# KangWelly/Assignment-for-AAE6102_GNSS-SDR

Measured on AMD Instinct MI355X. Metric: correlator Msamples/s (acq+track), whole job, higher is better.
Workload: dtype int8 in; acquisition: f64 correlation + f64 fine search; tracking: f64

## Files before the change

assignment-for-aae6102_gnss-sdr_amd/abi.py:

```python
from __future__ import annotations

import ctypes as C
import os
import sys

MAX_SV = 64
MAX_TAPS = 32

OK, ENODATA, EIO, EARG, EDEVICE, EINDEX = 0, 1, 2, 3, 4, 5

FIELDS = ["P_i", "P_q", "E_i", "E_q", "L_i", "L_q", "PLLdiscri", "DLLdiscri", "codedelay",
          "remChip", "codeFreq", "carrierFreq", "remPhase", "remSample", "numSample",
          "delayValue", "absoluteSample", "codedelay2"]
NFIELDS = len(FIELDS)
OUT_DEVICE = 1
FIELDS_POS = ["P_i", "P_q", "E_i", "E_q", "L_i", "L_q", "carrError", "codeError", "codedelay",
              "remChip", "codeFreq", "carrFreq", "remCarrPhase", "absoluteSampleCodedelay",
              "numSample", "delayValue", "absoluteSample", "codedelay2"]

MC_TAPS = 25
MC_TAP_NAMES = ([f"E_{{}}{s}" for s in ["_060", "_055", "", "_045", "_040", "_035", "_030", "_025",
                                         "_020", "_015", "_010", "_005"]] + ["P_{}"] +
                [f"L_{{}}{s}" for s in ["005", "010", "015", "020", "025", "030", "035", "040", "045",
                                         "", "055", "060"]])
# ... 319 lines not shown
                                    C.POINTER(GnssAcfOut)]),
    "gnss_acf_fit": (C.c_int, [C.c_void_p, C.POINTER(GnssAcfFitCfg), C.POINTER(GnssTrackOut), C.c_int32,
                               C.POINTER(GnssAcfFitOut)]),
    "gnss_acf_fit_window": (C.c_int, [C.POINTER(GnssAcfFitCfg), C.POINTER(C.c_double), C.POINTER(C.c_double),
                                      C.POINTER(GnssAcfFitOut)]),
    "gnss_lane_boundaries": (C.c_int, [C.POINTER(C.c_double), C.POINTER(C.c_double), C.c_int, C.c_int, C.c_double]),
    "gnss_ctx_lane_path": (C.c_int, [C.c_void_p]),
}

LIB_PATH = os.path.join(os.path.dirname(os.path.abspath(__file__)), "lib", "libgnss_mi355x.so")
_lib = None
_torch_first = False
LOADED_PATH = None

(OPT_FORCE_SUB, OPT_NO_PERSIST, OPT_FORCE_VPB, OPT_ACQ_ROCFFT, OPT_FINE_ROCFFT, OPT_ACQ_BATCH, OPT_ACQ_FUSED,
 OPT_ACQ_RING, OPT_ACQ_PIPE, OPT_VT_BLOCKS, OPT_FORCE_PEER, OPT_VT_SPAN, OPT_SLOT_PATH) = range(13)
MAX_DEVICES = 16


def require_torch():
    import torch
    if _lib is not None and not _torch_first:
        raise RuntimeError("import torch before the first gnss Context / abi.load() "
                           "(PyTorch-ROCm must bring up its HIP runtime first)")
    return torch


class GnssError(RuntimeError):
    def __init__(self, status, msg=""):
        self.status = status
        super().__init__(f"gnss status {status}: {msg}")
# ... 31 lines not shown
```

assignment-for-aae6102_gnss-sdr_amd/csrc/acq_fft.hip:

```cpp
#include "gnss_internal.h"

#pragma clang fp contract(fast)

namespace gnss {

namespace {

constexpr int kRow = 2000;
constexpr int kRowPad = 2100;
constexpr int kRowThreads = 256;
constexpr int kColThreads = 256;

template <int P> struct PrimeTab;
template <> struct PrimeTab<13> {
    static constexpr double c[13] = {1.0, 0.8854560256532099, 0.5680647467311559, 0.120536680255323, -0.35460488704253545, -0.7485107481711012, -0.970941817426052, -0.9709418174260521, -0.7485107481711013, -0.3546048870425359, 0.1205366802553232, 0.5680647467311548, 0.88545602565321};
    static constexpr double s[13] = {0.0, 0.4647231720437685, 0.8229838658936564, 0.992708874098054, 0.9350162426854148, 0.6631226582407952, 0.23931566428755768, -0.23931566428755743, -0.663122658240795, -0.9350162426854147, -0.992708874098054, -0.822983865893657, -0.4647231720437684};
};
template <> struct PrimeTab<29> {
    static constexpr double c[29] = {1.0, 0.9766205557100867, 0.907575419670957, 0.7960930657056438, 0.6473862847818277, 0.46840844069979015, 0.26752833852922075, 0.05413890858541761, -0.16178199655276473, -0.37013815533991423, -0.5611870653623823, -0.7259954919231306, -0.8568571761675893, -0.9476531711828025, -0.9941379571543596, -0.9941379571543597, -0.9476531711828025, -0.8568571761675892, -0.7259954919231311, -0.5611870653623825, -0.37013815533991445, -0.16178199655276476, 0.0541389085854167, 0.2675283385292201, 0.4684084406997903, 0.6473862847818279, 0.796093065705644, 0.9075754196709569, 0.9766205557100867};
    static constexpr double s[29] = {0.0, 0.21497044021102407, 0.4198891015602646, 0.6051742151937652, 0.7621620551276365, 0.8835120444460229, 0.963549992519223, 0.9985334138511238, 0.9868265225415261, 0.9289767198167915, 0.8276889981568906, 0.6876994588534235, 0.5155538571770216, 0.3193015301359798, 0.10811901842394192, -0.10811901842394124, -0.31930153013597995, -0.5155538571770218, -0.6876994588534231, -0.8276889981568905, -0.9289767198167914, -0.9868265225415261, -0.9985334138511239, -0.9635499925192231, -0.8835120444460228, -0.7621620551276362, -0.6051742151937649, -0.41988910156026493, -0.21497044021102438};
};

template <class V> struct RealOf;
template <> struct RealOf<float2> { using T = float; };
// ... 905 lines not shown
    t[e] = tw_row[t2 ? 10 * i * k : i * k];
}

__device__ __forceinline__ int64_t fine_code_of(int64_t n, double invFs, double invFc, double codelength)
{
    const double cvi = floor((invFs * (double)(n + 1)) / invFc);
    return (int64_t)fmod(cvi, codelength);
}

#ifndef GNSS_FINE_PREP
#define GNSS_FINE_PREP 1
#endif
#ifndef GNSS_FINE_TWIK
#define GNSS_FINE_TWIK 1
#endif
template <class Src> struct SrcElem;
template <> struct SrcElem<SrcIQ8> {
    using T = char2;
    static constexpr int kTM = 32;
    __device__ static T get(const SrcIQ8& s, int64_t n) { return reinterpret_cast<const char2*>(s.p)[n]; }
    static SrcIQ8 wrap(const T* p) { return SrcIQ8{reinterpret_cast<const int8_t*>(p)}; }
};
template <> struct SrcElem<SrcC64> {
    using T = double2;
    static constexpr int kTM = 8;
    __device__ static T get(const SrcC64& s, int64_t n) { return s.p[n]; }
    static SrcC64 wrap(const T* p) { return SrcC64{p}; }
};
template <int P, class Src>
__global__ __launch_bounds__(kRowThreads) void fine_prep_kernel(
    const Src src, const int32_t* __restrict__ cd, int64_t S, double invFs, double invFc, double codelength,
    const float* __restrict__ ca0, typename SrcElem<Src>::T* __restrict__ xt0, float* __restrict__ ct0)
{
    using T = typename SrcElem<Src>::T;
    constexpr int PT = P * kFineT, TM = SrcElem<Src>::kTM;
    constexpr int64_t M = (int64_t)PT * kRow;
    __shared__ T s_x[TM * PT];
    __shared__ float s_c[TM * PT];
    const float* ca = ca0 + (int64_t)blockIdx.y * 1023;
    const int m0 = blockIdx.x * TM, tid = threadIdx.x;
    const int tm = kRow - m0 < TM ? kRow - m0 : TM;
    const int64_t base = S - cd[blockIdx.y] - 1, n0 = (int64_t)PT * m0;
    for (int e = tid; e < tm * PT; e += kRowThreads) {
        s_x[e] = SrcElem<Src>::get(src, base + n0 + e);
        s_c[e] = ca[fine_code_of(n0 + e, invFs, invFc, codelength)];
    }
    __syncthreads();
    T* xt = xt0 + (int64_t)blockIdx.y * M;
    float* ct = ct0 + (int64_t)blockIdx.y * M;
    for (int e = tid; e < tm * PT; e += kRowThreads) {
        const int rho = e / tm, c = e - rho * tm;
        xt[(int64_t)rho * kRow + m0 + c] = s_x[c * PT + rho];
        ct[(int64_t)rho * kRow + m0 + c] = s_c[c * PT + rho];
    }
}

template <int P, class Src>
__global__ __launch_bounds__(kRowThreads) void fine_rows_kernel(
    const Src src, const float* __restrict__ ct, const int32_t* __restrict__ cd, int64_t S,
    const float* __restrict__ ca0, double invFs, double invFc, double codelength, int D, int64_t N,
    const double2* __restrict__ tw_row, const double2* __restrict__ twik, const double2* __restrict__ tabA,
    const double2* __restrict__ tabB, double2* __restrict__ E0)
{
    constexpr int T = kFineT;
    const int64_t base = S - cd[blockIdx.z] - 1;
    const float* ca = ca0 + (int64_t)blockIdx.z * 1023;
    double2* E = E0 + (int64_t)blockIdx.z * N;
    __shared__ double2 s_a[kRowPad];
    const int rho = blockIdx.x, r = blockIdx.y, tid = threadIdx.x;
    const int m2 = rho / P, n2 = rho - m2 * P;
    auto sample = [&](int m1) { return (int64_t)P * T * m1 + (int64_t)P * m2 + n2; };
    auto code_of = [&](int64_t n) { return fine_code_of(n, invFs, invFc, codelength); };
    if constexpr (GNSS_FINE_PREP) {
        constexpr int NIT = (kRow + kRowThreads - 1) / kRowThreads;
        const int64_t row0 = ((int64_t)blockIdx.z * P * T + rho) * kRow;
        double2 raw[NIT], ta[NIT];
        float cv[NIT];
#pragma unroll
        for (int q = 0; q < NIT; q++) {
            const int m10 = tid + q * kRowThreads, m1 = m10 < kRow ? m10 : kRow - 1;
            cv[q] = ct[row0 + m1];
// ... 49 lines not shown
        fft2000_r20first_put<-1>(s_a, tw_row, tid, put);
}

struct FineBest {
    double m;
    int64_t i;
};

__device__ __forceinline__ void best_merge(double& m, int64_t& i, double m2, int64_t i2)
{
    if (m2 > m || (m2 == m && i2 < i)) { m = m2; i = i2; }
}

template <int P>
__global__ __launch_bounds__(kColThreads) void fine_cols_kernel(
    const double2* __restrict__ E0, int D, int64_t N, int shifted, const double2* __restrict__ tabK,
    const double2* __restrict__ tabS, FineBest* __restrict__ part0)
{
    constexpr int T = kFineT, JC = kFineJC;
    const double2* E = E0 + (int64_t)blockIdx.z * N;
    FineBest* part = part0 + (int64_t)blockIdx.z * gridDim.x * gridDim.y;
    static_assert(P * T * JC * sizeof(double2) + (kColThreads / 64) * sizeof(double) * 2 <= 80 * 1024,
                  "fine_cols LDS tile: two blocks per CU of gfx950's 160 KiB");
    __shared__ double2 s_e[P * T * JC];
    __shared__ FineBest s_b[kColThreads / 64];
    const int r = blockIdx.y, j10 = blockIdx.x * JC, tid = threadIdx.x;
    auto at = [&](int e) {
        const int jj = e % JC, nm = e / JC;
        return E + ((int64_t)r * P * T + nm) * kRow + j10 + jj;
    };
    if constexpr (GNSS_STAGED_LOADS) {
        constexpr int NE = P * T * JC, NIT = (NE + kColThreads - 1) / kColThreads;
        double2 st[NIT];
#pragma unroll
// ... 40 lines not shown
    }
#pragma unroll
    for (int o = 32; o > 0; o >>= 1) {
        const double m2 = __shfl_xor(bm, o, 64);
        const int64_t i2 = __shfl_xor(bi, o, 64);
        best_merge(bm, bi, m2, i2);
    }
    if ((tid & 63) == 0) s_b[tid >> 6] = FineBest{bm, bi};
    __syncthreads();
    if (tid == 0) {
        for (int w = 1; w < kColThreads / 64; w++) best_merge(bm, bi, s_b[w].m, s_b[w].i);
        part[(int64_t)r * gridDim.x + blockIdx.x] = FineBest{bm, bi};
    }
}

__global__ void fine_best_final_kernel(const FineBest* __restrict__ part0, int nblk,
                                       int64_t* __restrict__ kbest0)
{
    const FineBest* part = part0 + (int64_t)blockIdx.x * nblk;
    int64_t* kbest = kbest0 + blockIdx.x;
    double bm = -1.0;
    int64_t bi = INT64_MAX;
    for (int k = threadIdx.x; k < nblk; k += blockDim.x) best_merge(bm, bi, part[k].m, part[k].i);
#pragma unroll
    for (int o = 32; o > 0; o >>= 1) {
        const double m2 = __shfl_xor(bm, o, 64);
        const int64_t i2 = __shfl_xor(bi, o, 64);
        best_merge(bm, bi, m2, i2);
    }
    __shared__ FineBest s_b[4];
    if ((threadIdx.x & 63) == 0) s_b[threadIdx.x >> 6] = FineBest{bm, bi};
    __syncthreads();
    if (threadIdx.x == 0) {
        for (int w = 1; w < (int)(blockDim.x >> 6); w++) best_merge(bm, bi, s_b[w].m, s_b[w].i);
        *kbest = bi + 1;
    }
}

}

bool acq_fft_supported(int64_t S) { return S == 13 * kRow || S == 29 * kRow; }

template <class V>
hipError_t launch_acq_fft_forward(const int8_t* iq, const double2* xs, int64_t S, int datalen, int nbins,
                                  double IF, double freqMin, double freqStep, double Fs, const float* ca,
                                  int nprn, double codeFreqBasis, const V* tw_row,
                                  const V* tw_col, V* B, V* X, hipStream_t s, int bin0, int nbc, bool codes)
{
    const int nsig = datalen * nbins;
    if (nbc < 0) nbc = nbins - bin0;
    if (bin0 < 0 || nbc < 0 || bin0 + nbc > nbins) return hipErrorInvalidValue;
// ... 136 lines not shown
};
FineLayout fine_layout(int64_t S, int L, int datalen)
{
    FineLayout f;
    f.M = (int64_t)L * S;
    f.N = f.M * datalen;
    f.tabs = kRow + (int64_t)kRow * datalen + (int64_t)kFineT * kRow + S + f.M / kRow + kTwIK;
    f.slab = f.N;
    f.part = (int64_t)datalen * (kRow / kFineJC);
    return f;
}
}

static size_t fine_prep_offset(const FineLayout& f, int nsv)
{
    const size_t b = sizeof(double2) * (size_t)(f.tabs + (int64_t)nsv * f.slab) + sizeof(FineBest) * (size_t)(nsv * f.part);
    return (b + 255) & ~(size_t)255;
}
size_t fine_fft_scratch_bytes(int64_t S, int L, int datalen, int nsv)
{
    const FineLayout f = fine_layout(S, L, datalen);
    if (!GNSS_FINE_PREP) return fine_prep_offset(f, nsv);
    return fine_prep_offset(f, nsv) + (size_t)nsv * f.M * (sizeof(double2) + sizeof(float));
}

hipError_t launch_fine_fft_tables(int64_t S, int L, int datalen, void* scratch, hipStream_t s)
{
    const int64_t M = (int64_t)L * S;
    double2* tw_row = static_cast<double2*>(scratch);
    double2* tabA = tw_row + kRow;
    double2* tabB = tabA + (int64_t)kRow * datalen;
    double2* tabK = tabB + (int64_t)kFineT * kRow;
    double2* tabS = tabK + S;
    const int64_t lens[5] = {kRow, (int64_t)kRow * datalen, (int64_t)kFineT * kRow, S, M / kRow};
    const int64_t divs[5] = {kRow, (int64_t)kRow * datalen, (int64_t)kFineT * kRow, M, M / kRow};
    const int64_t rows[5] = {0, kRow, kRow, kRow, 0};
    double2* tabs[5] = {tw_row, tabA, tabB, tabK, tabS};
    for (int t = 0; t < 5; t++)
        hipLaunchKernelGGL(fine_twiddle_kernel, dim3((unsigned)((lens[t] + 255) / 256)), dim3(256), 0,
                           s, tabs[t], lens[t], divs[t], rows[t]);
    hipLaunchKernelGGL(fine_twik_kernel, dim3((kTwIK + 255) / 256), dim3(256), 0, s, tw_row, tabS + M / kRow);
    return hipGetLastError();
}

hipError_t launch_fine_fft_argmax(const int8_t* iq, const double2* xs, int64_t S, int L, int datalen,
                                  const int32_t* cd, int nsv, const float* ca, double Fs, double codeFreqBasis,
                                  double codelength, int shifted, void* scratch, int64_t* kbest, hipStream_t s)
{
    if (nsv < 1 || nsv > 65535) return hipErrorInvalidValue;
    const FineLayout f = fine_layout(S, L, datalen);
    const int64_t N = f.N;
    double2* tw_row = static_cast<double2*>(scratch);
    double2* tabA = tw_row + kRow;
    double2* tabB = tabA + (int64_t)kRow * datalen;
    double2* tabK = tabB + (int64_t)kFineT * kRow;
    double2* tabS = tabK + S;
    double2* E = tw_row + f.tabs;
    FineBest* part = reinterpret_cast<FineBest*>(E + (int64_t)nsv * f.slab);
    char* prep = static_cast<char*>(scratch) + fine_prep_offset(f, nsv);
    float* ct = reinterpret_cast<float*>(prep + (size_t)nsv * f.M * sizeof(double2));
    const int nblk = kRow / kFineJC;
    auto rows = [&](auto src, auto* xt, auto kern, auto prep_kern, int tm) {
        using SrcT = decltype(src);
        if (GNSS_FINE_PREP) {
            hipLaunchKernelGGL(prep_kern, dim3((kRow + tm - 1) / tm, nsv), dim3(kRowThreads), 0, s, src, cd, S, 1 / Fs,
                               1 / codeFreqBasis, codelength, ca, xt, ct);
            src = SrcElem<SrcT>::wrap(xt);
        }
        hipLaunchKernelGGL(kern, dim3((unsigned)(f.M / kRow), datalen, nsv), dim3(kRowThreads), 0, s, src, ct, cd, S,
                           ca, 1 / Fs, 1 / codeFreqBasis, codelength, datalen, N, tw_row, tabS + f.M / kRow, tabA,
                           tabB, E);
    };
#define GNSS_FINE(P_)                                                                           \
    if (S == (int64_t)P_ * kRow) {                                                              \
        if (xs)                                                                                 \
            rows(SrcC64{xs}, reinterpret_cast<double2*>(prep), fine_rows_kernel<P_, SrcC64>,    \
                 fine_prep_kernel<P_, SrcC64>, SrcElem<SrcC64>::kTM);                           \
        else                                                                                    \
            rows(SrcIQ8{iq}, reinterpret_cast<char2*>(prep), fine_rows_kernel<P_, SrcIQ8>,      \
                 fine_prep_kernel<P_, SrcIQ8>, SrcElem<SrcIQ8>::kTM);                           \
        hipLaunchKernelGGL(fine_cols_kernel<P_>, dim3(nblk, datalen, nsv), dim3(kColThreads), 0, s, E, \
                           datalen, N, shifted, tabK, tabS, part);                                    \
        hipLaunchKernelGGL(fine_best_final_kernel, dim3(nsv), dim3(256), 0, s, part, nblk * datalen, \
                           kbest);                                                              \
        return hipGetLastError();                                                               \
    }
    GNSS_FINE(13) GNSS_FINE(29)
#undef GNSS_FINE
    return hipErrorInvalidValue;
}

}
```

assignment-for-aae6102_gnss-sdr_amd/csrc/api_acq.cpp:

```cpp
#include <cmath>
#include <cstring>
#include <vector>

#include "host.h"

using namespace gnss;
using namespace gnss::host;

namespace {
constexpr int kAcqPipeDefault = 2;
#ifndef GNSS_ACQ_FWD_SPLIT
#define GNSS_ACQ_FWD_SPLIT 1
#endif
constexpr bool kAcqFwdSplit = GNSS_ACQ_FWD_SPLIT;
constexpr int kAcqPairFront = 60;
constexpr int kFineBatch = 16;

template <class V> struct CplxReal;
template <> struct CplxReal<float2> { using T = float; };
template <> struct CplxReal<double2> { using T = double; };

template <class V>
int acq_search(gnss_ctx* ctx, const int8_t* blk, const double2* xa, int64_t S, int dl, int nb, int np,
               const gnss_signal* sg, const gnss_acq* acq, const float* ca, typename CplxReal<V>::T* corr,
// ... 145 lines not shown
    for (int p0 = 0; p0 < np; p0 += chunk) {
        const int pc = std::min(chunk, np - p0);
        if ((st = get_plan(ctx, S, (size_t)pc * nsig, dbl, 1, &pl))) return st;
    }
    HIP_TRY(hipEventRecord(e_all.a, ctx->stream));
    HIP_TRY(launch_acq_wipe(blk, xa, S, dl, nb, sg->IF, acq->freqMin, acq->freqStep, sg->Fs, sig.as<V>(), ctx->stream));
    if ((st = run_fft(ctx, sig.p, S, nsig, dbl, 0))) return st;
    HIP_TRY(launch_acq_code(ca, nullptr, np, S, sg->codeFreqBasis, sg->Fs, code.as<V>(), ctx->stream));
    if ((st = run_fft(ctx, code.p, S, np, dbl, 0))) return st;
    for (int p0 = 0; p0 < np; p0 += chunk) {
        const int pc = std::min(chunk, np - p0);
        HIP_TRY(launch_acq_mul(code.as<V>() + (size_t)p0 * S, sig.as<V>(), pc, nsig, S, y.as<V>(), ctx->stream));
        if ((st = run_fft(ctx, y.p, S, (size_t)pc * nsig, dbl, 1))) return st;
        HIP_TRY(launch_acq_power(y.as<V>(), pc, nb, dl, S, 0, corr + (size_t)p0 * nb * S, ctx->stream));
    }
    return GNSS_OK;
}
}

static int group_acquisition(gnss_ctx* g, const gnss_file* file, const gnss_signal* sg, const gnss_acq* acq,
                             gnss_acquired* out, gnss_acq_diag* diag)
{
    if (!file || !sg || !acq || !out) return GNSS_EARG;
    memset(out, 0, sizeof(*out));
    if (diag) memset(diag, 0, sizeof(*diag));
    g->timing = gnss_timing{};
    std::vector<int32_t> prns;
    if (acq->n_prn > 0 && acq->prn_list) prns.assign(acq->prn_list, acq->prn_list + acq->n_prn);
    else for (int i = 1; i <= 32; i++) prns.push_back(i);
    if (prns.size() > GNSS_MAX_SV) return fail(g, GNSS_EARG, "too many PRNs");
// ... 84 lines not shown
                                     xs_sums.as<unsigned long long>() + 2, ctx->stream));
        HIP_TRY(hipEventRecord(e_conv.b, ctx->stream));
    }
    const double2* xa = iq8 ? nullptr : xs_acq.as<double2>();
    const double2* xf = iq8 ? nullptr : xs_fine.as<double2>();

    std::vector<float> cah((size_t)np * 1023);
    for (int i = 0; i < np; i++) generate_ca(prns[i], &cah[(size_t)i * 1023]);
    DevBuf ca, corr, peaks, scratch;
    HIP_TRY(ca.alloc(ctx, "acq.ca", cah.size() * sizeof(float)));
    HIP_TRY(hipMemcpyAsync(ca.p, cah.data(), cah.size() * sizeof(float), hipMemcpyHostToDevice, ctx->stream));
    const int dbl = ctx->acq_fp64 ? 1 : 0;
    HIP_TRY(corr.alloc(ctx, "acq.corr", (dbl ? sizeof(double) : sizeof(float)) * (size_t)np * nb * S));
    HIP_TRY(peaks.alloc(ctx, "acq.peaks", sizeof(AcqPeak) * (size_t)np));
    HIP_TRY(scratch.alloc(ctx, "acq.scratch", acq_scratch_bytes(np, np)));
    Events e_all, e_corr;
    int perm = 0;
    DevBuf fsync;
    if (dbl)
        st = acq_search<double2>(ctx, blk, xa, S, dl, nb, np, sg, acq, ca.as<float>(), corr.as<double>(), e_all,
                                 &perm, fsync);
    else
        st = acq_search<float2>(ctx, blk, xa, S, dl, nb, np, sg, acq, ca.as<float>(), corr.as<float>(), e_all,
                                &perm, fsync);
    if (st) return st;
    const int cshift = (int)std::ceil(sg->Fs / sg->codeFreqBasis);
    if (dbl)
        HIP_TRY(launch_acq_peak(corr.as<double>(), np, nb, S, cshift, perm, peaks.as<AcqPeak>(), scratch.p,
                                ctx->stream));
    else
        HIP_TRY(launch_acq_peak(corr.as<float>(), np, nb, S, cshift, perm, peaks.as<AcqPeak>(), scratch.p,
                                ctx->stream));
    HIP_TRY(hipEventRecord(e_corr.b, ctx->stream));
    std::vector<AcqPeak> ph((size_t)np);
    HIP_TRY(hipMemcpyAsync(ph.data(), peaks.p, sizeof(AcqPeak) * (size_t)np, hipMemcpyDeviceToHost, ctx->stream));
    unsigned fused_err = 0;
    if (fsync.p)
        HIP_TRY(hipMemcpyAsync(&fused_err, static_cast<char*>(fsync.p) + acq_fused_err_offset(), sizeof(unsigned),
                               hipMemcpyDeviceToHost, ctx->stream));
    HIP_TRY(hipStreamSynchronize(ctx->stream));
    if (fused_err)
        return fail(ctx, GNSS_EDEVICE, "fused correlator: a pipeline wait timed out (grid not resident)");
    ctx->timing.acq_hypothesis_samples = (int64_t)np * nb * dl * S;

    std::vector<int> acq_idx;
    for (int i = 0; i < np; i++) {
        if (diag) {
            int k = diag->n++;
            diag->prn[k] = prns[i];
            diag->SNR[k] = ph[i].snr;
            diag->fbin[k] = ph[i].fbin + 1;
            diag->codePhase[k] = ph[i].cp + 1;
            diag->peak[k] = ph[i].peak;
            diag->peak2[k] = ph[i].peak2;
        }
        if (ph[i].snr >= 12) {
            int k = out->n++;
            out->sv[k] = prns[i];
            out->SNR[k] = ph[i].snr;
            out->Doppler[k] = acq->freqMin + acq->freqStep * (double)ph[i].fbin;
            out->codedelay[k] = ph[i].cp;
            acq_idx.push_back(i);
        }
    }
    if (out->n == 0) {
        HIP_TRY(hipEventRecord(e_all.b, ctx->stream));
        HIP_TRY(hipEventSynchronize(e_all.b));
        ctx->timing.acq_ms = e_all.ms();
        ctx->timing.acq_corr_ms = ctx->timing.acq_ms;
        return fail(ctx, GNSS_ENODATA, "No satellites acquired");
    }

    if (flen < off + S * bps * (L + 1)) return fail(ctx, GNSS_EIO, "IF record too short for fine search");
    const int fshift = dtyp == 2 ? 1 : 2;
    const int na = out->n;
    const int64_t N = (int64_t)L * S * dl;
    if (N % 2) return fail(ctx, GNSS_EINDEX, "odd fftlength: MATLAB indexes past the end (:116)");
    std::vector<float> caf((size_t)na * 1023);
    std::vector<int32_t> cdh((size_t)na);
    for (int k = 0; k < na; k++) {
        generate_ca(out->sv[k], &caf[(size_t)k * 1023]);
        cdh[k] = out->codedelay[k];
    }
    DevBuf fca, fcd, fx, kb;
    HIP_TRY(fca.alloc(ctx, "acq.fca", caf.size() * sizeof(float)));
    HIP_TRY(fcd.alloc(ctx, "acq.fcd", cdh.size() * sizeof(int32_t)));
    HIP_TRY(kb.alloc(ctx, "acq.kb", sizeof(int64_t) * (size_t)na));
    HIP_TRY(hipMemcpyAsync(fca.p, caf.data(), caf.size() * sizeof(float), hipMemcpyHostToDevice, ctx->stream));
    HIP_TRY(hipMemcpyAsync(fcd.p, cdh.data(), cdh.size() * sizeof(int32_t), hipMemcpyHostToDevice, ctx->stream));
    const bool own_fine = fine_fft_supported(S, L) && !ctx->opt[GNSS_OPT_FINE_ROCFFT];
    Events e_fine;
    if (own_fine) {
        const int fb = std::min(na, kFineBatch);
        HIP_TRY(fx.alloc(ctx, "acq.fx", fine_fft_scratch_bytes(S, L, dl, fb)));
        HIP_TRY(hipEventRecord(e_fine.a, ctx->stream));
        HIP_TRY(launch_fine_fft_tables(S, L, dl, fx.p, ctx->stream));
        for (int k0 = 0; k0 < na; k0 += fb) {
            const int nk = std::min(fb, na - k0);
            HIP_TRY(launch_fine_fft_argmax(blk, xf, S, L, dl, fcd.as<int32_t>() + k0, nk,
                                           fca.as<float>() + (size_t)k0 * 1023, sg->Fs, sg->codeFreqBasis,
                                           sg->codelength, fshift, fx.p, kb.as<int64_t>() + k0, ctx->stream));
        }
    } else {
        HIP_TRY(fx.alloc(ctx, "acq.fx", sizeof(double2) * (size_t)na * N));
        rocfft_plan pl;
        if ((st = get_plan(ctx, N, na, 1, 0, &pl))) return st;
        HIP_TRY(hipEventRecord(e_fine.a, ctx->stream));
        HIP_TRY(launch_fine_build(blk, xf, S, L, fcd.as<int32_t>(), fca.as<float>(), na, sg->Fs, sg->codeFreqBasis,
                                  sg->codelength, N, fx.as<double2>(), ctx->stream));
        if ((st = run_fft(ctx, fx.p, N, na, 1, 0))) return st;
        DevBuf fscr;
        HIP_TRY(fscr.alloc(ctx, "acq.fscr", acq_scratch_bytes(1, na)));
        HIP_TRY(launch_fine_argmax(fx.as<double2>(), na, N, fshift, fscr.p, kb.as<int64_t>(), ctx->stream));
    }
    HIP_TRY(hipEventRecord(e_fine.b, ctx->stream));
    HIP_TRY(hipEventRecord(e_all.b, ctx->stream));
    std::vector<int64_t> kh((size_t)na);
    HIP_TRY(hipMemcpyAsync(kh.data(), kb.p, sizeof(int64_t) * (size_t)na, hipMemcpyDeviceToHost, ctx->stream));
    HIP_TRY(hipStreamSynchronize(ctx->stream));
    for (int k = 0; k < na; k++) {
        const double K = (double)kh[k];
        out->fineFreq[k] = (file->dataType == 2) ? (-K * (sg->Fs / (double)N) + sg->Fs / 2) : (K * (sg->Fs / (double)N));
    }
    {
        float f = 0;
        (void)hipEventElapsedTime(&f, e_all.a, e_corr.b);
        ctx->timing.acq_corr_ms = f;
    }
    ctx->timing.acq_fine_ms = e_fine.ms();
    ctx->timing.acq_ms = e_all.ms() + (iq8 ? 0.0 : e_conv.ms());
    return GNSS_OK;
}

}
// ... 1 lines not shown
```

assignment-for-aae6102_gnss-sdr_amd/csrc/gnss_internal.h:

```cpp
#pragma once

#include <hip/hip_runtime.h>
#include <stdint.h>

#include "../../include/gnss_mi355x.h"

#define GNSS_HD __host__ __device__ __forceinline__

namespace gnss {

struct Colon {
    double a, d, c;
    int64_t n;
};

GNSS_HD Colon colon_make(double a, double d, double b)
{
    Colon r{a, d, b, -1};
    if (!(a - a == 0) || !(d - d == 0) || !(b - b == 0)) return r;
    if (d == 0 || (a < b && d < 0) || (b < a && d > 0)) return r;
    double tol = 2.0 * 2.220446049250313e-16 * fmax(fabs(a), fabs(b));
    double sig = d > 0 ? 1.0 : -1.0;
    double n;
    if (a == floor(a) && d == 1) {
// ... 400 lines not shown
hipError_t launch_acq_fft_correlate(const double2* C, const double2* X, int64_t S, int datalen,
                                    int nbins, int nprn, int first_pair, int npair,
                                    const double2* tw_row, const double2* tw_col, double2* A,
                                    double* corr, hipStream_t s, int parts = kAcqCols | kAcqRows);
hipError_t launch_acq_fft_pair(const double2* C, const double2* X, int64_t S, int datalen, int nbins, int nprn,
                               int cols_first, int cols_n, double2* Acols, int rows_first, int rows_n,
                               const double2* Arows, const double2* tw_row, const double2* tw_col, double* corr,
                               int front, hipStream_t s);
size_t acq_fused_sync_bytes();
size_t acq_fused_err_offset();
size_t acq_fused_ring_bytes(int64_t S);
hipError_t launch_acq_fft_correlate_fused(const double2* C, const double2* X, int64_t S, int datalen, int nbins,
                                          int nprn, int nslot, const double2* tw_row, const double2* tw_col,
                                          double2* ring, void* sync, double* corr, hipStream_t s);
bool fine_fft_supported(int64_t S, int L);
size_t fine_fft_scratch_bytes(int64_t S, int L, int datalen, int nsv);
hipError_t launch_fine_fft_tables(int64_t S, int L, int datalen, void* scratch, hipStream_t s);
hipError_t launch_fine_fft_argmax(const int8_t* iq, const double2* xs, int64_t S, int L, int datalen,
                                  const int32_t* cd, int nsv, const float* ca, double Fs, double codeFreqBasis,
                                  double codelength, int shifted, void* scratch, int64_t* kbest, hipStream_t s);
hipError_t launch_fine_build(const int8_t* iq, const double2* xs, int64_t S, int L, const int32_t* codedelay,
                             const float* ca, int nsv, double Fs, double codeFreqBasis,
                             double codelength, int64_t N, double2* out, hipStream_t s);
hipError_t launch_fine_argmax(const double2* F, int nsv, int64_t N, int shifted, void* scratch,
                              int64_t* kbest, hipStream_t s);

size_t acq_scratch_bytes(int nprn, int nsv);

hipError_t launch_stage_cpx(const int8_t* src, int prec, int type, int64_t nsamp, double2* out,
                            unsigned long long* sums, hipStream_t s);
hipError_t launch_real8_to_iq8(const int8_t* src, int64_t n, int8_t* dst, hipStream_t s);
size_t prefix16_scratch_bytes(int64_t ngroups);
hipError_t launch_prefix16(const short* src, int64_t ngroups, long long* pref_i, long long* pref_q,
                           void* scratch, size_t scratch_bytes, hipStream_t s);

// ... 265 lines not shown
```

assignment-for-aae6102_gnss-sdr_amd/csrc/host.h:

```cpp
#pragma once

#include <hip/hip_runtime.h>
#include <rocfft/rocfft.h>

#include <algorithm>
#include <cstdint>
#include <cstdlib>
#include <map>
#include <string>
#include <thread>
#include <tuple>
#include <utility>
#include <vector>

#include "gnss_internal.h"
#include "group.h"

struct gnss_ctx {
    int device = 0;
    hipStream_t stream = nullptr;
    hipStream_t stream2 = nullptr;
    hipEvent_t ev_cols[2] = {}, ev_rows[2] = {};
    std::string err;
    gnss_timing timing{};
    int profiling = 0;
    std::map<std::tuple<size_t, size_t, int, int>, rocfft_plan> plans;
    void* fft_work = nullptr;
    size_t fft_work_size = 0;
    std::map<std::string, std::pair<void*, size_t>> pool;
    std::map<std::string, std::pair<void*, size_t>> pinned;
    int64_t acq_tw_S = 0;
    int acq_tw_dbl = -1;
    int acq_fp64 = 1;
    uint64_t window = 0;
    int64_t opt[GNSS_OPT_COUNT] = {};
    int lane_path = 0;
    std::vector<gnss_ctx*> members;
    bool member = false;
    int fail_chan = -1;
    gnss::group::ResidentCache<void*> resident;
};

namespace gnss {
namespace host {

inline const char* probe_env(const char* name)
{
// ... 136 lines not shown
```

include/gnss_mi355x.h:

```cpp
#ifndef GNSS_MI355X_H
#define GNSS_MI355X_H

#include <stdint.h>
#include <stddef.h>

#ifdef __cplusplus
extern "C" {
#endif

#define GNSS_ABI_VERSION 13

#define GNSS_OK         0
#define GNSS_ENODATA    1
#define GNSS_EIO        2
#define GNSS_EARG       3
#define GNSS_EDEVICE    4
#define GNSS_EINDEX     5

#define GNSS_MAX_SV     64
#define GNSS_MAX_TAPS   32


typedef struct gnss_file {
    const char   *path;
// ... 119 lines not shown
int  gnss_ctx_set_acq_precision(gnss_ctx *ctx, int fp64);
int  gnss_ctx_set_window(gnss_ctx *ctx, uint64_t bytes);
#define GNSS_OPT_FORCE_SUB    0
#define GNSS_OPT_NO_PERSIST   1
#define GNSS_OPT_FORCE_VPB    2
#define GNSS_OPT_ACQ_ROCFFT   3
#define GNSS_OPT_FINE_ROCFFT  4
#define GNSS_OPT_ACQ_BATCH    5
#define GNSS_OPT_ACQ_FUSED    6
#define GNSS_OPT_ACQ_RING     7
#define GNSS_OPT_ACQ_PIPE     8
#define GNSS_OPT_VT_BLOCKS    9
#define GNSS_OPT_FORCE_PEER   10
#define GNSS_OPT_VT_SPAN      11
#define GNSS_OPT_SLOT_PATH    12
#define GNSS_OPT_COUNT        13
int  gnss_ctx_set_option(gnss_ctx *ctx, int key, int64_t value);
int  gnss_lane_boundaries(const double *taps, const double *post, int n_taps, int lane_samples,
                          double cps_max);
int  gnss_ctx_lane_path(const gnss_ctx *ctx);

int  gnss_dev_alloc(gnss_ctx *ctx, uint64_t nbytes, void **dev_ptr);
int  gnss_dev_free(gnss_ctx *ctx, void *dev_ptr);
int  gnss_dev_upload(gnss_ctx *ctx, void *dev_dst, const void *host_src, uint64_t nbytes);
int  gnss_dev_download(gnss_ctx *ctx, void *host_dst, const void *dev_src, uint64_t nbytes);

int gnss_acquisition(gnss_ctx *ctx, const gnss_file *file, const gnss_signal *signal,
                     const gnss_acq *acq, gnss_acquired *out, gnss_acq_diag *diag);

int gnss_tracking_ct(gnss_ctx *ctx, const gnss_file *file, const gnss_signal *signal,
                     const gnss_track *track, const gnss_acquired *acquired,
// ... 374 lines not shown
```

Before: 401,000.

## Select acquired SVs on device and launch first fine-search batch before host sync

```diff
diff --git a/assignment-for-aae6102_gnss-sdr_amd/abi.py b/assignment-for-aae6102_gnss-sdr_amd/abi.py
--- a/assignment-for-aae6102_gnss-sdr_amd/abi.py
+++ b/assignment-for-aae6102_gnss-sdr_amd/abi.py
@@ -357,7 +357,8 @@
 LOADED_PATH = None
 
 (OPT_FORCE_SUB, OPT_NO_PERSIST, OPT_FORCE_VPB, OPT_ACQ_ROCFFT, OPT_FINE_ROCFFT, OPT_ACQ_BATCH, OPT_ACQ_FUSED,
- OPT_ACQ_RING, OPT_ACQ_PIPE, OPT_VT_BLOCKS, OPT_FORCE_PEER, OPT_VT_SPAN, OPT_SLOT_PATH) = range(13)
+ OPT_ACQ_RING, OPT_ACQ_PIPE, OPT_VT_BLOCKS, OPT_FORCE_PEER, OPT_VT_SPAN, OPT_SLOT_PATH,
+ OPT_FINE_HOST_ORDER) = range(14)
 MAX_DEVICES = 16
 
 
diff --git a/assignment-for-aae6102_gnss-sdr_amd/csrc/acq_fft.hip b/assignment-for-aae6102_gnss-sdr_amd/csrc/acq_fft.hip
--- a/assignment-for-aae6102_gnss-sdr_amd/csrc/acq_fft.hip
+++ b/assignment-for-aae6102_gnss-sdr_amd/csrc/acq_fft.hip
@@ -943,6 +943,12 @@
 #ifndef GNSS_FINE_TWIK
 #define GNSS_FINE_TWIK 1
 #endif
+struct FineSel {
+    const int32_t* list;
+    const int32_t* cd;
+    int k0;
+};
+
 template <class Src> struct SrcElem;
 template <> struct SrcElem<SrcIQ8> {
     using T = char2;
@@ -958,7 +964,7 @@
 };
 template <int P, class Src>
 __global__ __launch_bounds__(kRowThreads) void fine_prep_kernel(
-    const Src src, const int32_t* __restrict__ cd, int64_t S, double invFs, double invFc, double codelength,
+    const Src src, const FineSel sel, int64_t S, double invFs, double invFc, double codelength,
     const float* __restrict__ ca0, typename SrcElem<Src>::T* __restrict__ xt0, float* __restrict__ ct0)
 {
     using T = typename SrcElem<Src>::T;
@@ -966,10 +972,12 @@
     constexpr int64_t M = (int64_t)PT * kRow;
     __shared__ T s_x[TM * PT];
     __shared__ float s_c[TM * PT];
-    const float* ca = ca0 + (int64_t)blockIdx.y * 1023;
+    const int sv = sel.k0 + blockIdx.y;
+    if (sv >= sel.list[0]) return;
+    const float* ca = ca0 + (int64_t)sel.list[1 + sv] * 1023;
     const int m0 = blockIdx.x * TM, tid = threadIdx.x;
     const int tm = kRow - m0 < TM ? kRow - m0 : TM;
-    const int64_t base = S - cd[blockIdx.y] - 1, n0 = (int64_t)PT * m0;
+    const int64_t base = S - sel.cd[sv] - 1, n0 = (int64_t)PT * m0;
     for (int e = tid; e < tm * PT; e += kRowThreads) {
         s_x[e] = SrcElem<Src>::get(src, base + n0 + e);
         s_c[e] = ca[fine_code_of(n0 + e, invFs, invFc, codelength)];
@@ -986,14 +994,16 @@
 
 template <int P, class Src>
 __global__ __launch_bounds__(kRowThreads) void fine_rows_kernel(
-    const Src src, const float* __restrict__ ct, const int32_t* __restrict__ cd, int64_t S,
+    const Src src, const float* __restrict__ ct, const FineSel sel, int64_t S,
     const float* __restrict__ ca0, double invFs, double invFc, double codelength, int D, int64_t N,
     const double2* __restrict__ tw_row, const double2* __restrict__ twik, const double2* __restrict__ tabA,
     const double2* __restrict__ tabB, double2* __restrict__ E0)
 {
     constexpr int T = kFineT;
-    const int64_t base = S - cd[blockIdx.z] - 1;
-    const float* ca = ca0 + (int64_t)blockIdx.z * 1023;
+    const int sv = sel.k0 + blockIdx.z;
+    if (sv >= sel.list[0]) return;
+    const int64_t base = S - sel.cd[sv] - 1;
+    const float* ca = ca0 + (int64_t)sel.list[1 + sv] * 1023;
     double2* E = E0 + (int64_t)blockIdx.z * N;
     __shared__ double2 s_a[kRowPad];
     const int rho = blockIdx.x, r = blockIdx.y, tid = threadIdx.x;
@@ -1073,10 +1083,11 @@
 
 template <int P>
 __global__ __launch_bounds__(kColThreads) void fine_cols_kernel(
-    const double2* __restrict__ E0, int D, int64_t N, int shifted, const double2* __restrict__ tabK,
-    const double2* __restrict__ tabS, FineBest* __restrict__ part0)
+    const double2* __restrict__ E0, const FineSel sel, int D, int64_t N, int shifted,
+    const double2* __restrict__ tabK, const double2* __restrict__ tabS, FineBest* __restrict__ part0)
 {
     constexpr int T = kFineT, JC = kFineJC;
+    if (sel.k0 + (int)blockIdx.z >= sel.list[0]) return;
     const double2* E = E0 + (int64_t)blockIdx.z * N;
     FineBest* part = part0 + (int64_t)blockIdx.z * gridDim.x * gridDim.y;
     static_assert(P * T * JC * sizeof(double2) + (kColThreads / 64) * sizeof(double) * 2 <= 80 * 1024,
@@ -1147,11 +1158,13 @@
     }
 }
 
-__global__ void fine_best_final_kernel(const FineBest* __restrict__ part0, int nblk,
+__global__ void fine_best_final_kernel(const FineBest* __restrict__ part0, int nblk, const FineSel sel,
                                        int64_t* __restrict__ kbest0)
 {
+    const int sv = sel.k0 + blockIdx.x;
+    if (sv >= sel.list[0]) return;
     const FineBest* part = part0 + (int64_t)blockIdx.x * nblk;
-    int64_t* kbest = kbest0 + blockIdx.x;
+    int64_t* kbest = kbest0 + sv;
     double bm = -1.0;
     int64_t bi = INT64_MAX;
     for (int k = threadIdx.x; k < nblk; k += blockDim.x) best_merge(bm, bi, part[k].m, part[k].i);
@@ -1168,6 +1181,20 @@
         for (int w = 1; w < (int)(blockDim.x >> 6); w++) best_merge(bm, bi, s_b[w].m, s_b[w].i);
         *kbest = bi + 1;
     }
+}
+
+__global__ void fine_select_kernel(const AcqPeak* __restrict__ peaks, int np, int32_t* __restrict__ list,
+                                   int32_t* __restrict__ cd)
+{
+    if (blockIdx.x || threadIdx.x) return;
+    int n = 0;
+    for (int i = 0; i < np; i++)
+        if (peaks[i].snr >= 12) {
+            list[1 + n] = i;
+            cd[n] = peaks[i].cp;
+            n++;
+        }
+    list[0] = n;
 }
 
 }
@@ -1334,8 +1361,12 @@
 
 static size_t fine_prep_offset(const FineLayout& f, int nsv)
 {
-    const size_t b = sizeof(double2) * (size_t)(f.tabs + (int64_t)nsv * f.slab) + sizeof(FineBest) * (size_t)(nsv * f.part);
+    const size_t b = sizeof(double2) * (size_t)((int64_t)nsv * f.slab) + sizeof(FineBest) * (size_t)(nsv * f.part);
     return (b + 255) & ~(size_t)255;
+}
+size_t fine_fft_tables_bytes(int64_t S, int L, int datalen)
+{
+    return sizeof(double2) * (size_t)fine_layout(S, L, datalen).tabs;
 }
 size_t fine_fft_scratch_bytes(int64_t S, int L, int datalen, int nsv)
 {
@@ -1344,10 +1375,10 @@
     return fine_prep_offset(f, nsv) + (size_t)nsv * f.M * (sizeof(double2) + sizeof(float));
 }
 
-hipError_t launch_fine_fft_tables(int64_t S, int L, int datalen, void* scratch, hipStream_t s)
+hipError_t launch_fine_fft_tables(int64_t S, int L, int datalen, void* tables, hipStream_t s)
 {
     const int64_t M = (int64_t)L * S;
-    double2* tw_row = static_cast<double2*>(scratch);
+    double2* tw_row = static_cast<double2*>(tables);
     double2* tabA = tw_row + kRow;
     double2* tabB = tabA + (int64_t)kRow * datalen;
     double2* tabK = tabB + (int64_t)kFineT * kRow;
@@ -1363,31 +1394,39 @@
     return hipGetLastError();
 }
 
+hipError_t launch_fine_select(const AcqPeak* peaks, int np, int32_t* list, int32_t* cd, hipStream_t s)
+{
+    hipLaunchKernelGGL(fine_select_kernel, dim3(1), dim3(64), 0, s, peaks, np, list, cd);
+    return hipGetLastError();
+}
+
 hipError_t launch_fine_fft_argmax(const int8_t* iq, const double2* xs, int64_t S, int L, int datalen,
-                                  const int32_t* cd, int nsv, const float* ca, double Fs, double codeFreqBasis,
-                                  double codelength, int shifted, void* scratch, int64_t* kbest, hipStream_t s)
-{
-    if (nsv < 1 || nsv > 65535) return hipErrorInvalidValue;
+                                  const int32_t* list, const int32_t* cd, int k0, int nsv, const float* ca,
+                                  double Fs, double codeFreqBasis, double codelength, int shifted,
+                                  const void* tables, void* scratch, int64_t* kbest, hipStream_t s)
+{
+    if (nsv < 1 || nsv > 65535 || k0 < 0) return hipErrorInvalidValue;
     const FineLayout f = fine_layout(S, L, datalen);
     const int64_t N = f.N;
-    double2* tw_row = static_cast<double2*>(scratch);
-    double2* tabA = tw_row + kRow;
-    double2* tabB = tabA + (int64_t)kRow * datalen;
-    double2* tabK = tabB + (int64_t)kFineT * kRow;
-    double2* tabS = tabK + S;
-    double2* E = tw_row + f.tabs;
+    const double2* tw_row = static_cast<const double2*>(tables);
+    const double2* tabA = tw_row + kRow;
+    const double2* tabB = tabA + (int64_t)kRow * datalen;
+    const double2* tabK = tabB + (int64_t)kFineT * kRow;
+    const double2* tabS = tabK + S;
+    double2* E = static_cast<double2*>(scratch);
     FineBest* part = reinterpret_cast<FineBest*>(E + (int64_t)nsv * f.slab);
     char* prep = static_cast<char*>(scratch) + fine_prep_offset(f, nsv);
     float* ct = reinterpret_cast<float*>(prep + (size_t)nsv * f.M * sizeof(double2));
     const int nblk = kRow / kFineJC;
+    const FineSel sel{list, cd, k0};
     auto rows = [&](auto src, auto* xt, auto kern, auto prep_kern, int tm) {
         using SrcT = decltype(src);
         if (GNSS_FINE_PREP) {
-            hipLaunchKernelGGL(prep_kern, dim3((kRow + tm - 1) / tm, nsv), dim3(kRowThreads), 0, s, src, cd, S, 1 / Fs,
+            hipLaunchKernelGGL(prep_kern, dim3((kRow + tm - 1) / tm, nsv), dim3(kRowThreads), 0, s, src, sel, S, 1 / Fs,
                                1 / codeFreqBasis, codelength, ca, xt, ct);
             src = SrcElem<SrcT>::wrap(xt);
         }
-        hipLaunchKernelGGL(kern, dim3((unsigned)(f.M / kRow), datalen, nsv), dim3(kRowThreads), 0, s, src, ct, cd, S,
+        hipLaunchKernelGGL(kern, dim3((unsigned)(f.M / kRow), datalen, nsv), dim3(kRowThreads), 0, s, src, ct, sel, S,
                            ca, 1 / Fs, 1 / codeFreqBasis, codelength, datalen, N, tw_row, tabS + f.M / kRow, tabA,
                            tabB, E);
     };
@@ -1399,9 +1438,9 @@
         else                                                                                    \
             rows(SrcIQ8{iq}, reinterpret_cast<char2*>(prep), fine_rows_kernel<P_, SrcIQ8>,      \
                  fine_prep_kernel<P_, SrcIQ8>, SrcElem<SrcIQ8>::kTM);                           \
-        hipLaunchKernelGGL(fine_cols_kernel<P_>, dim3(nblk, datalen, nsv), dim3(kColThreads), 0, s, E, \
-                           datalen, N, shifted, tabK, tabS, part);                                    \
-        hipLaunchKernelGGL(fine_best_final_kernel, dim3(nsv), dim3(256), 0, s, part, nblk * datalen, \
+        hipLaunchKernelGGL(fine_cols_kernel<P_>, dim3(nblk, datalen, nsv), dim3(kColThreads), 0, s, E, sel, \
+                           datalen, N, shifted, tabK, tabS, part);                              \
+        hipLaunchKernelGGL(fine_best_final_kernel, dim3(nsv), dim3(256), 0, s, part, nblk * datalen, sel, \
                            kbest);                                                              \
         return hipGetLastError();                                                               \
     }
diff --git a/assignment-for-aae6102_gnss-sdr_amd/csrc/api_acq.cpp b/assignment-for-aae6102_gnss-sdr_amd/csrc/api_acq.cpp
--- a/assignment-for-aae6102_gnss-sdr_amd/csrc/api_acq.cpp
+++ b/assignment-for-aae6102_gnss-sdr_amd/csrc/api_acq.cpp
@@ -183,6 +183,20 @@
         if ((st = run_fft(ctx, y.p, S, (size_t)pc * nsig, dbl, 1))) return st;
         HIP_TRY(launch_acq_power(y.as<V>(), pc, nb, dl, S, 0, corr + (size_t)p0 * nb * S, ctx->stream));
     }
+    return GNSS_OK;
+}
+
+int fine_tables(gnss_ctx* ctx, int64_t S, int L, int dl, DevBuf& t)
+{
+    HIP_TRY(t.alloc(ctx, "acq.ftab", fine_fft_tables_bytes(S, L, dl)));
+    if (ctx->fine_tab_p == t.p && ctx->fine_tab_S == S && ctx->fine_tab_L == L && ctx->fine_tab_dl == dl)
+        return GNSS_OK;
+    ctx->fine_tab_p = nullptr;
+    HIP_TRY(launch_fine_fft_tables(S, L, dl, t.p, ctx->stream));
+    ctx->fine_tab_p = t.p;
+    ctx->fine_tab_S = S;
+    ctx->fine_tab_L = L;
+    ctx->fine_tab_dl = dl;
     return GNSS_OK;
 }
 }
@@ -297,7 +311,30 @@
     HIP_TRY(corr.alloc(ctx, "acq.corr", (dbl ? sizeof(double) : sizeof(float)) * (size_t)np * nb * S));
     HIP_TRY(peaks.alloc(ctx, "acq.peaks", sizeof(AcqPeak) * (size_t)np));
     HIP_TRY(scratch.alloc(ctx, "acq.scratch", acq_scratch_bytes(np, np)));
-    Events e_all, e_corr;
+    const int64_t N = (int64_t)L * S * dl;
+    const bool fine_len = flen >= off + S * bps * (L + 1);
+    const bool own_fine = fine_fft_supported(S, L) && !ctx->opt[GNSS_OPT_FINE_ROCFFT];
+    const int fshift = dtyp == 2 ? 1 : 2;
+    DevBuf fx, ftab, fsel, fcd, kb;
+    HIP_TRY(fsel.alloc(ctx, "acq.fsel", sizeof(int32_t) * (size_t)(np + 1)));
+    HIP_TRY(fcd.alloc(ctx, "acq.fcd", sizeof(int32_t) * (size_t)np));
+    HIP_TRY(kb.alloc(ctx, "acq.kb", sizeof(int64_t) * (size_t)np));
+    bool dev_order = own_fine && fine_len && N % 2 == 0 && !ctx->opt[GNSS_OPT_FINE_HOST_ORDER];
+    int fb = 0;
+    if (dev_order) {
+        fb = std::min(np, kFineBatch);
+        if (fx.alloc(ctx, "acq.fx", fine_fft_scratch_bytes(S, L, dl, fb)) != hipSuccess) {
+            (void)hipGetLastError();
+            dev_order = false;
+        }
+    }
+    if (own_fine && fine_len && (st = fine_tables(ctx, S, L, dl, ftab))) return st;
+    auto fine_batch = [&](int k0, int nk) {
+        return launch_fine_fft_argmax(blk, xf, S, L, dl, fsel.as<int32_t>(), fcd.as<int32_t>(), k0, nk,
+                                      ca.as<float>(), sg->Fs, sg->codeFreqBasis, sg->codelength, fshift, ftab.p,
+                                      fx.p, kb.as<int64_t>(), ctx->stream);
+    };
+    Events e_all, e_corr, e_fine;
     int perm = 0;
     DevBuf fsync;
     if (dbl)
@@ -316,6 +353,17 @@
                                 ctx->stream));
     HIP_TRY(hipEventRecord(e_corr.b, ctx->stream));
     std::vector<AcqPeak> ph((size_t)np);
+    std::vector<int32_t> selh((size_t)np + 1, 0);
+    std::vector<int64_t> kh((size_t)np);
+    if (dev_order) {
+        HIP_TRY(launch_fine_select(peaks.as<AcqPeak>(), np, fsel.as<int32_t>(), fcd.as<int32_t>(), ctx->stream));
+        HIP_TRY(hipEventRecord(e_fine.a, ctx->stream));
+        HIP_TRY(fine_batch(0, fb));
+        HIP_TRY(hipEventRecord(e_fine.b, ctx->stream));
+        HIP_TRY(hipEventRecord(e_all.b, ctx->stream));
+        HIP_TRY(hipMemcpyAsync(selh.data(), fsel.p, sizeof(int32_t) * selh.size(), hipMemcpyDeviceToHost, ctx->stream));
+        HIP_TRY(hipMemcpyAsync(kh.data(), kb.p, sizeof(int64_t) * (size_t)fb, hipMemcpyDeviceToHost, ctx->stream));
+    }
     HIP_TRY(hipMemcpyAsync(ph.data(), peaks.p, sizeof(AcqPeak) * (size_t)np, hipMemcpyDeviceToHost, ctx->stream));
     unsigned fused_err = 0;
     if (fsync.p)
@@ -326,7 +374,7 @@
         return fail(ctx, GNSS_EDEVICE, "fused correlator: a pipeline wait timed out (grid not resident)");
     ctx->timing.acq_hypothesis_samples = (int64_t)np * nb * dl * S;
 
-    std::vector<int> acq_idx;
+    std::vector<int32_t> acq_idx, cdh;
     for (int i = 0; i < np; i++) {
         if (diag) {
             int k = diag->n++;
@@ -344,63 +392,64 @@
             out->Doppler[k] = acq->freqMin + acq->freqStep * (double)ph[i].fbin;
             out->codedelay[k] = ph[i].cp;
             acq_idx.push_back(i);
-        }
-    }
-    if (out->n == 0) {
-        HIP_TRY(hipEventRecord(e_all.b, ctx->stream));
-        HIP_TRY(hipEventSynchronize(e_all.b));
+            cdh.push_back(ph[i].cp);
+        }
+    }
+    const int na = out->n;
+    if (dev_order && (selh[0] != na || !std::equal(acq_idx.begin(), acq_idx.end(), selh.begin() + 1)))
+        return fail(ctx, GNSS_EDEVICE, "fine search: the device's list of acquired SVs is not the host's");
+    if (na == 0) {
+        if (!dev_order) {
+            HIP_TRY(hipEventRecord(e_all.b, ctx->stream));
+            HIP_TRY(hipEventSynchronize(e_all.b));
+        }
         ctx->timing.acq_ms = e_all.ms();
         ctx->timing.acq_corr_ms = ctx->timing.acq_ms;
         return fail(ctx, GNSS_ENODATA, "No satellites acquired");
     }
 
-    if (flen < off + S * bps * (L + 1)) return fail(ctx, GNSS_EIO, "IF record too short for fine search");
-    const int fshift = dtyp == 2 ? 1 : 2;
-    const int na = out->n;
-    const int64_t N = (int64_t)L * S * dl;
+    if (!fine_len) return fail(ctx, GNSS_EIO, "IF record too short for fine search");
     if (N % 2) return fail(ctx, GNSS_EINDEX, "odd fftlength: MATLAB indexes past the end (:116)");
-    std::vector<float> caf((size_t)na * 1023);
-    std::vector<int32_t> cdh((size_t)na);
-    for (int k = 0; k < na; k++) {
-        generate_ca(out->sv[k], &caf[(size_t)k * 1023]);
-        cdh[k] = out->codedelay[k];
-    }
-    DevBuf fca, fcd, fx, kb;
-    HIP_TRY(fca.alloc(ctx, "acq.fca", caf.size() * sizeof(float)));
-    HIP_TRY(fcd.alloc(ctx, "acq.fcd", cdh.size() * sizeof(int32_t)));
-    HIP_TRY(kb.alloc(ctx, "acq.kb", sizeof(int64_t) * (size_t)na));
-    HIP_TRY(hipMemcpyAsync(fca.p, caf.data(), caf.size() * sizeof(float), hipMemcpyHostToDevice, ctx->stream));
-    HIP_TRY(hipMemcpyAsync(fcd.p, cdh.data(), cdh.size() * sizeof(int32_t), hipMemcpyHostToDevice, ctx->stream));
-    const bool own_fine = fine_fft_supported(S, L) && !ctx->opt[GNSS_OPT_FINE_ROCFFT];
-    Events e_fine;
-    if (own_fine) {
-        const int fb = std::min(na, kFineBatch);
-        HIP_TRY(fx.alloc(ctx, "acq.fx", fine_fft_scratch_bytes(S, L, dl, fb)));
-        HIP_TRY(hipEventRecord(e_fine.a, ctx->stream));
-        HIP_TRY(launch_fine_fft_tables(S, L, dl, fx.p, ctx->stream));
-        for (int k0 = 0; k0 < na; k0 += fb) {
-            const int nk = std::min(fb, na - k0);
-            HIP_TRY(launch_fine_fft_argmax(blk, xf, S, L, dl, fcd.as<int32_t>() + k0, nk,
-                                           fca.as<float>() + (size_t)k0 * 1023, sg->Fs, sg->codeFreqBasis,
-                                           sg->codelength, fshift, fx.p, kb.as<int64_t>() + k0, ctx->stream));
-        }
+    int done = 0;
+    if (dev_order) {
+        done = std::min(na, fb);
+        for (int k0 = done; k0 < na; k0 += fb) HIP_TRY(fine_batch(k0, std::min(fb, na - k0)));
     } else {
-        HIP_TRY(fx.alloc(ctx, "acq.fx", sizeof(double2) * (size_t)na * N));
-        rocfft_plan pl;
-        if ((st = get_plan(ctx, N, na, 1, 0, &pl))) return st;
-        HIP_TRY(hipEventRecord(e_fine.a, ctx->stream));
-        HIP_TRY(launch_fine_build(blk, xf, S, L, fcd.as<int32_t>(), fca.as<float>(), na, sg->Fs, sg->codeFreqBasis,
-                                  sg->codelength, N, fx.as<double2>(), ctx->stream));
-        if ((st = run_fft(ctx, fx.p, N, na, 1, 0))) return st;
-        DevBuf fscr;
-        HIP_TRY(fscr.alloc(ctx, "acq.fscr", acq_scratch_bytes(1, na)));
-        HIP_TRY(launch_fine_argmax(fx.as<double2>(), na, N, fshift, fscr.p, kb.as<int64_t>(), ctx->stream));
-    }
-    HIP_TRY(hipEventRecord(e_fine.b, ctx->stream));
-    HIP_TRY(hipEventRecord(e_all.b, ctx->stream));
-    std::vector<int64_t> kh((size_t)na);
-    HIP_TRY(hipMemcpyAsync(kh.data(), kb.p, sizeof(int64_t) * (size_t)na, hipMemcpyDeviceToHost, ctx->stream));
-    HIP_TRY(hipStreamSynchronize(ctx->stream));
+        selh[0] = na;
+        std::copy(acq_idx.begin(), acq_idx.end(), selh.begin() + 1);
+        HIP_TRY(hipMemcpyAsync(fsel.p, selh.data(), sizeof(int32_t) * (size_t)(na + 1), hipMemcpyHostToDevice,
+                               ctx->stream));
+        HIP_TRY(hipMemcpyAsync(fcd.p, cdh.data(), sizeof(int32_t) * (size_t)na, hipMemcpyHostToDevice, ctx->stream));
+        if (own_fine) {
+            fb = std::min(na, kFineBatch);
+            HIP_TRY(fx.alloc(ctx, "acq.fx", fine_fft_scratch_bytes(S, L, dl, fb)));
+            HIP_TRY(hipEventRecord(e_fine.a, ctx->stream));
+            for (int k0 = 0; k0 < na; k0 += fb) HIP_TRY(fine_batch(k0, std::min(fb, na - k0)));
+        } else {
+            std::vector<float> caf((size_t)na * 1023);
+            for (int k = 0; k < na; k++) generate_ca(out->sv[k], &caf[(size_t)k * 1023]);
+            DevBuf fca;
+            HIP_TRY(fca.alloc(ctx, "acq.fca", caf.size() * sizeof(float)));
+            HIP_TRY(hipMemcpyAsync(fca.p, caf.data(), caf.size() * sizeof(float), hipMemcpyHostToDevice, ctx->stream));
+            HIP_TRY(fx.alloc(ctx, "acq.fx", sizeof(double2) * (size_t)na * N));
+            rocfft_plan pl;
+            if ((st = get_plan(ctx, N, na, 1, 0, &pl))) return st;
+            HIP_TRY(hipEventRecord(e_fine.a, ctx->stream));
+            HIP_TRY(launch_fine_build(blk, xf, S, L, fcd.as<int32_t>(), fca.as<float>(), na, sg->Fs,
+                                      sg->codeFreqBasis, sg->codelength, N, fx.as<double2>(), ctx->stream));
+            if ((st = run_fft(ctx, fx.p, N, na, 1, 0))) return st;
+            DevBuf fscr;
+            HIP_TRY(fscr.alloc(ctx, "acq.fscr", acq_scratch_bytes(1, na)));
+            HIP_TRY(launch_fine_argmax(fx.as<double2>(), na, N, fshift, fscr.p, kb.as<int64_t>(), ctx->stream));
+        }
+    }
+    if (done < na) {
+        HIP_TRY(hipEventRecord(e_fine.b, ctx->stream));
+        HIP_TRY(hipEventRecord(e_all.b, ctx->stream));
+        HIP_TRY(hipMemcpyAsync(kh.data() + done, kb.as<int64_t>() + done, sizeof(int64_t) * (size_t)(na - done),
+                               hipMemcpyDeviceToHost, ctx->stream));
+        HIP_TRY(hipStreamSynchronize(ctx->stream));
+    }
     for (int k = 0; k < na; k++) {
         const double K = (double)kh[k];
         out->fineFreq[k] = (file->dataType == 2) ? (-K * (sg->Fs / (double)N) + sg->Fs / 2) : (K * (sg->Fs / (double)N));
diff --git a/assignment-for-aae6102_gnss-sdr_amd/csrc/gnss_internal.h b/assignment-for-aae6102_gnss-sdr_amd/csrc/gnss_internal.h
--- a/assignment-for-aae6102_gnss-sdr_amd/csrc/gnss_internal.h
+++ b/assignment-for-aae6102_gnss-sdr_amd/csrc/gnss_internal.h
@@ -438,11 +438,14 @@
                                           int nprn, int nslot, const double2* tw_row, const double2* tw_col,
                                           double2* ring, void* sync, double* corr, hipStream_t s);
 bool fine_fft_supported(int64_t S, int L);
+size_t fine_fft_tables_bytes(int64_t S, int L, int datalen);
+hipError_t launch_fine_fft_tables(int64_t S, int L, int datalen, void* tables, hipStream_t s);
+hipError_t launch_fine_select(const AcqPeak* peaks, int np, int32_t* list, int32_t* cd, hipStream_t s);
 size_t fine_fft_scratch_bytes(int64_t S, int L, int datalen, int nsv);
-hipError_t launch_fine_fft_tables(int64_t S, int L, int datalen, void* scratch, hipStream_t s);
 hipError_t launch_fine_fft_argmax(const int8_t* iq, const double2* xs, int64_t S, int L, int datalen,
-                                  const int32_t* cd, int nsv, const float* ca, double Fs, double codeFreqBasis,
-                                  double codelength, int shifted, void* scratch, int64_t* kbest, hipStream_t s);
+                                  const int32_t* list, const int32_t* cd, int k0, int nsv, const float* ca,
+                                  double Fs, double codeFreqBasis, double codelength, int shifted,
+                                  const void* tables, void* scratch, int64_t* kbest, hipStream_t s);
 hipError_t launch_fine_build(const int8_t* iq, const double2* xs, int64_t S, int L, const int32_t* codedelay,
                              const float* ca, int nsv, double Fs, double codeFreqBasis,
                              double codelength, int64_t N, double2* out, hipStream_t s);
diff --git a/assignment-for-aae6102_gnss-sdr_amd/csrc/host.h b/assignment-for-aae6102_gnss-sdr_amd/csrc/host.h
--- a/assignment-for-aae6102_gnss-sdr_amd/csrc/host.h
+++ b/assignment-for-aae6102_gnss-sdr_amd/csrc/host.h
@@ -31,6 +31,9 @@
     std::map<std::string, std::pair<void*, size_t>> pinned;
     int64_t acq_tw_S = 0;
     int acq_tw_dbl = -1;
+    const void* fine_tab_p = nullptr;
+    int64_t fine_tab_S = 0;
+    int fine_tab_L = 0, fine_tab_dl = 0;
     int acq_fp64 = 1;
     uint64_t window = 0;
     int64_t opt[GNSS_OPT_COUNT] = {};
diff --git a/include/gnss_mi355x.h b/include/gnss_mi355x.h
--- a/include/gnss_mi355x.h
+++ b/include/gnss_mi355x.h
@@ -157,7 +157,8 @@
 #define GNSS_OPT_FORCE_PEER   10
 #define GNSS_OPT_VT_SPAN      11
 #define GNSS_OPT_SLOT_PATH    12
-#define GNSS_OPT_COUNT        13
+#define GNSS_OPT_FINE_HOST_ORDER 13
+#define GNSS_OPT_COUNT        14
 int  gnss_ctx_set_option(gnss_ctx *ctx, int key, int64_t value);
 int  gnss_lane_boundaries(const double *taps, const double *post, int n_taps, int lane_samples,
                           double cps_max);
```

After: 399,400. No clear change (-0.4%).
